# lucagiorgetti/Laplace-DQN-Snake-game

Hardware: NVIDIA B200
Metric: snake_env_steps_per_sec (higher is better)
Workload: dtype u64 bitboards -> f32 obs

## Files before the change

### include/snake_b200.h

```cpp
#ifndef SNAKE_B200_H
#define SNAKE_B200_H

#include <stddef.h>
#include <stdint.h>

#ifdef __cplusplus
extern "C" {
#endif

#define SNK_VERSION 200

#if defined(__GNUC__)
#define SNK_API __attribute__((visibility("default")))
#else
#define SNK_API
#endif

#define SNK_OK 0
#define SNK_ERR_INVALID (-1)
#define SNK_ERR_CUDA (-2)
#define SNK_ERR_NODEVICE (-3)
#define SNK_ERR_UNSUPPORTED (-4)
#define SNK_ERR_TIMEOUT (-5)

// ... 10 lines not shown
#define SNK_OBS_BITS 5

typedef struct snk_env *snk_handle;

SNK_API int snk_create(snk_handle *out, int64_t n_envs, int device, uint32_t flags);
SNK_API int snk_destroy(snk_handle h);
SNK_API int snk_reset(snk_handle h);
SNK_API int snk_set_food_list_host(snk_handle h, const uint8_t *cells_rc_host, int n);
SNK_API int snk_default_food_list_host(uint8_t *cells_rc_host , int *n);
SNK_API int snk_set_stream(snk_handle h, void *cuda_stream);
SNK_API int snk_use_own_stream(snk_handle h);
SNK_API int snk_get_stream(snk_handle h, void **cuda_stream);
SNK_API int snk_set_seed(snk_handle h, uint64_t seed);
SNK_API int snk_sync(snk_handle h);
SNK_API int64_t snk_num_envs(snk_handle h);
SNK_API const char *snk_last_error(void);
SNK_API int snk_version(void);

SNK_API int snk_available_actions(snk_handle h, uint8_t *dirs_3xN);
SNK_API int snk_available_actions_host(snk_handle h, uint8_t *dirs_3xN_host);

SNK_API int snk_step(snk_handle h, const uint8_t *act_idx, float *reward, uint8_t *done);
SNK_API int snk_step_abs(snk_handle h, const uint8_t *dir, float *reward, uint8_t *done);

SNK_API int snk_step_fused(snk_handle h, const float *q, float eps, const float *u, const uint8_t *ridx,
                   uint8_t *act_idx, float *reward, uint8_t *done, void *obs, int obs_fmt,
                   uint8_t *mask, float *ep_return, int32_t *ep_score);
SNK_API int snk_step_fused_host(snk_handle h, const float *q, float eps, const float *u, const uint8_t *ridx,
                        uint8_t *act_idx, float *reward, uint8_t *done, void *obs, int obs_fmt,
                        uint8_t *mask, float *ep_return, int32_t *ep_score);
SNK_API int snk_rollout_fused(snk_handle h, const uint8_t *act_TxN, int64_t T, int is_abs, float *reward, uint8_t *done,
                              void *obs, int obs_fmt, uint8_t *mask, float *ep_return, int32_t *ep_score);
SNK_API int snk_debug_rollout_timing(long long *device_buf);
SNK_API int snk_host_alloc(void **p, size_t bytes);
SNK_API int snk_host_free(void *p);
#define SNK_ALLOC_COMPRESSIBLE 1u
SNK_API int snk_device_alloc(void **p, size_t bytes, int device, uint32_t flags, int *compressible);
SNK_API int snk_device_free(void *p);
SNK_API int snk_compression_supported(int device, int *yes);

SNK_API int snk_state(snk_handle h, void *obs, int obs_fmt);
SNK_API int snk_state_host(snk_handle h, void *obs_host, int obs_fmt);
SNK_API int snk_patch_reset_obs(snk_handle h, const uint8_t *done, void *obs, int obs_fmt);

SNK_API int snk_losing_mask(snk_handle h, uint8_t *mask_3xN);
SNK_API int snk_losing_mask_host(snk_handle h, uint8_t *mask_3xN_host);

SNK_API int snk_select_action(snk_handle h, const float *q_3xN, float eps, const float *u, const uint8_t *ridx,
                      uint8_t *act_idx_out);

SNK_API int snk_masked_target(const float *q_next_3xB, const uint8_t *mask_3xB, const float *r, const uint8_t *done,
                      double gamma, float fill, double *y_f64, float *y_f32, int64_t B, void *cuda_stream);

SNK_API int snk_get_score(snk_handle h, int32_t *score);
SNK_API int snk_get_done(snk_handle h, uint8_t *done);
SNK_API int snk_get_error_flags(snk_handle h, uint8_t *flags);
SNK_API int snk_get_steps(snk_handle h, int32_t *steps);
SNK_API int snk_get_score_host(snk_handle h, int32_t *score_host);
SNK_API int snk_get_done_host(snk_handle h, uint8_t *done_host);
SNK_API int snk_get_error_flags_host(snk_handle h, uint8_t *flags_host);
SNK_API int snk_get_steps_host(snk_handle h, int32_t *steps_host);
SNK_API int snk_count_errors_host(snk_handle h, int64_t *count);

SNK_API int snk_env_checkpoint_bytes(snk_handle h, size_t *bytes);
SNK_API int snk_env_save_host(snk_handle h, void *blob_host, size_t bytes);
SNK_API int snk_env_load_host(snk_handle h, const void *blob_host, size_t bytes, int64_t *first_bad_env);
// ... 105 lines not shown
```

### laplace-dqn-snake-game_b200/__init__.py

```python
import ctypes as C
import os
import warnings

import torch

_HERE = os.path.dirname(os.path.abspath(__file__))
LIB_PATH = os.environ.get("SNAKE_B200_LIB", os.path.join(_HERE, "libsnake_b200.so"))

OBS_NONE, OBS_F32, OBS_I8, OBS_I64, OBS_PACKED2, OBS_BITS = 0, 1, 2, 3, 4, 5
AUTO_RESET = 1
ENV_ERR_FOOD, ENV_ERR_ACTION = 1, 2
_OBS = {
    "f32": (OBS_F32, torch.float32, 200), "i8": (OBS_I8, torch.int8, 200),
    "i64": (OBS_I64, torch.int64, 200), "packed2": (OBS_PACKED2, torch.uint8, 50),
    "bits": (OBS_BITS, torch.uint8, 24),
}


def _obs_shape(fmt, lead):
    per = _OBS[fmt][2]
    return (*lead, 2, 10, 10) if per == 200 else (*lead, per)


def _fmt_code(out):
# ... 44 lines not shown
U, D, L, R = 0, 1, 2, 3
DIRS = ((-1, 0), (1, 0), (0, -1), (0, 1))


class SnakeB200Error(RuntimeError):
    pass


_lib = None


def lib():
    global _lib
    if _lib is not None:
        return _lib
    if not os.path.exists(LIB_PATH):
        raise SnakeB200Error(
            "%s not found: run `python -c 'import __graft_entry__ as g; g.build()'` (needs nvcc). "
            "There is no CPU fallback." % LIB_PATH)
    L = C.CDLL(LIB_PATH)
    vp, i64, u32, i32, f32, f64 = C.c_void_p, C.c_int64, C.c_uint32, C.c_int, C.c_float, C.c_double
    sig = {
        "snk_create": [C.POINTER(vp), i64, i32, u32],
        "snk_destroy": [vp], "snk_reset": [vp], "snk_sync": [vp],
        "snk_set_food_list_host": [vp, vp, i32],
        "snk_default_food_list_host": [vp, C.POINTER(i32)],
        "snk_set_stream": [vp, vp], "snk_use_own_stream": [vp], "snk_get_stream": [vp, C.POINTER(vp)],
        "snk_set_seed": [vp, C.c_uint64],
        "snk_available_actions": [vp, vp],
        "snk_step": [vp, vp, vp, vp], "snk_step_abs": [vp, vp, vp, vp],
        "snk_step_fused": [vp, vp, f32, vp, vp, vp, vp, vp, vp, i32, vp, vp, vp],
        "snk_step_fused_host": [vp, vp, f32, vp, vp, vp, vp, vp, vp, i32, vp, vp, vp],
        "snk_rollout_fused": [vp, vp, i64, i32, vp, vp, vp, i32, vp, vp, vp],
        "snk_host_alloc": [C.POINTER(vp), C.c_size_t], "snk_host_free": [vp],
        "snk_device_alloc": [C.POINTER(vp), C.c_size_t, i32, u32, C.POINTER(i32)], "snk_device_free": [vp],
        "snk_compression_supported": [i32, C.POINTER(i32)],
        "snk_state": [vp, vp, i32], "snk_losing_mask": [vp, vp],
        "snk_state_host": [vp, vp, i32], "snk_losing_mask_host": [vp, vp], "snk_available_actions_host": [vp, vp],
        "snk_patch_reset_obs": [vp, vp, vp, i32],
        "snk_get_score_host": [vp, vp], "snk_get_done_host": [vp, vp], "snk_get_error_flags_host": [vp, vp],
        "snk_get_steps_host": [vp, vp],
        "snk_step_fused_store_host": [vp, vp, vp, f32, vp, vp, vp, vp, vp, vp, i32, vp, vp, vp],
        "snk_replay_gather_host": [vp, vp, i64, vp, vp, vp, vp, vp, vp, vp],
        "snk_select_action": [vp, vp, f32, vp, vp, vp],
        "snk_masked_target": [vp, vp, vp, vp, f64, f32, vp, vp, i64, vp],
        "snk_get_score": [vp, vp], "snk_get_done": [vp, vp], "snk_get_error_flags": [vp, vp],
        "snk_get_steps": [vp, vp], "snk_count_errors_host": [vp, C.POINTER(i64)],
        "snk_env_checkpoint_bytes": [vp, C.POINTER(C.c_size_t)], "snk_env_save_host": [vp, vp, C.c_size_t],
        "snk_env_load_host": [vp, vp, C.c_size_t, C.POINTER(i64)],
        "snk_replay_checkpoint_bytes": [vp, C.POINTER(C.c_size_t)], "snk_replay_save_host": [vp, vp, C.c_size_t],
        "snk_replay_load_host": [vp, vp, C.c_size_t, C.POINTER(i64)],
        "snk_center_columns": [vp, i64, i64, vp, vp, vp],
        "snk_d_store_snapshot": [vp, i64, i64, i64, vp, vp],
        "snk_laplace_sample_weights": [vp, vp, vp, i64, i64, vp, vp, vp, vp],
        "snk_replay_create": [C.POINTER(vp), i64, i32], "snk_replay_destroy": [vp], "snk_replay_clear": [vp],
        "snk_replay_length": [vp, C.POINTER(i64), C.POINTER(i64)],
        "snk_step_fused_store": [vp, vp, vp, f32, vp, vp, vp, vp, vp, vp, i32, vp, vp, vp],
        "snk_replay_gather": [vp, vp, i64, vp, vp, vp, vp, vp, vp, vp, vp, vp],
        "snk_replay_sample_indices": [vp, C.c_uint64, i64, vp, vp],
        "snk_replay_bad_index_host": [vp, C.POINTER(i32)],
        "snk_qnet_create": [C.POINTER(vp), vp, i64, i32, i32], "snk_qnet_destroy": [vp],
        "snk_qnet_forward": [vp, vp, i64, vp, vp], "snk_qnet_precision": [vp, C.POINTER(i32)],
        "snk_qnet_overflow_host": [vp, C.POINTER(i32)], "snk_qnet_debug_timing": [vp, vp],
        "snk_qnet_sample_grads": [vp, vp, vp, vp, i64, vp, vp, i64, vp, i64, vp, vp],
        "snk_qnet_train_step": [vp, vp, vp, vp, i64, vp, f64, f64, f64, vp, vp, vp],
        "snk_qnet_set_params": [vp, vp, vp], "snk_qnet_params": [vp, C.POINTER(vp)],
# ... 496 lines not shown
```

### laplace-dqn-snake-game_b200/csrc/snake_env.cu

```cuda
#include <stdarg.h>
#include <string.h>

#include <new>
#include <mutex>
#include <type_traits>
#include <unordered_map>

#include <cuda.h>

#include "common.h"
#include "sm100.h"

#ifndef SNK_OBS_STORE_MODE
#define SNK_OBS_STORE_MODE 1
#endif
#if SNK_OBS_STORE_MODE == 1
#define SNK_OBS_STORE(p, v) (*(p) = (v))
#elif SNK_OBS_STORE_MODE == 2
#define SNK_OBS_STORE(p, v) __stwt((p), (v))
#else
#define SNK_OBS_STORE(p, v) __stcs((p), (v))
#endif

namespace snk {

static thread_local char g_err[512];
char *err_buf() { return g_err; }
int fail(int code, const char *fmt, ...) {
    va_list ap;
    va_start(ap, fmt);
    vsnprintf(g_err, sizeof(g_err), fmt, ap);
    va_end(ap);
    return code;
}

#ifndef SNK_TPB
#define SNK_TPB 256
#endif
#ifndef SNK_MINB
#define SNK_MINB 1
#endif
#ifndef SNK_UNROLL
#define SNK_UNROLL 4
#endif
constexpr int PHASE_B_UNROLL = SNK_UNROLL;
constexpr int TPB = SNK_TPB;
constexpr int MAX_FOOD = 64;
constexpr int PLANE_WORDS = 16;

constexpr int M_HR = 0, M_HC = 4, M_TR = 8, M_TC = 12, M_FR = 16, M_FC = 20, M_PFR = 24, M_PFC = 28;
constexpr int M_PD = 32, M_LEN = 34, M_T = 41, M_DONE = 51, M_ERR = 52;

constexpr u64 wall_bits(int lo_hi) {
    u64 lo = 0, hi = 0;
    for (int c = 0; c < 10; c++)
        for (int r = 0; r < 10; r++)
            if (r == 0 || r == 9 || c == 0 || c == 9) {
                int k = r + 10 * c;
                if (k < 64) lo |= 1ull << k; else hi |= 1ull << (k - 64);
            }
    return lo_hi ? hi : lo;
}
constexpr u64 WALL_LO = wall_bits(0), WALL_HI = wall_bits(1);

constexpr u64 INIT_OCC = (1ull << (6 + 0)) | (1ull << (7 + 0));
constexpr u64 INIT_MISC = (7ull << M_HR) | (1ull << M_HC) | (8ull << M_TR) | (1ull << M_TC) | (3ull << M_FR) |
                          (4ull << M_FC) | (3ull << M_PFR) | (4ull << M_PFC) | (0ull << M_PD) | (2ull << M_LEN);

struct FoodTable {
    uint8_t bit[MAX_FOOD];
    int n;
    __host__ __device__ u64 mask() const { return n >= 64 ? ~0ull : ((1ull << n) - 1ull); }
};
// ... 8 lines not shown
        case SNK_OBS_F32: return 800;
        case SNK_OBS_I8: return 200;
        case SNK_OBS_I64: return 1600;
        case SNK_OBS_PACKED2: return 50;
        case SNK_OBS_BITS: return 24;
        default: return 0;
    }
}

struct StepOutputs {
    float *reward;
    uint8_t *done;
    void *obs;
    uint8_t *mask;
    float *ep_return;
    int32_t *ep_score;
};

struct StepArgs {
    EnvState s;
    const uint8_t *act;
    const float *q;
    const float *u;
    const uint8_t *ridx;
    float eps;
    uint8_t *act_out;
    StepOutputs out;
    long long env_begin, env_end;
    u64 seed, step_counter;
    int auto_reset, is_abs;
    uint4 *sink;
    long long sink_base, sink_cap, sink_n;
    FoodTable food;
};

constexpr int REC_U4 = 8;

__host__ __device__ __forceinline__ u64 splitmix64(u64 x) {
    x += 0x9E3779B97F4A7C15ull;
    x = (x ^ (x >> 30)) * 0xBF58476D1CE4E5B9ull;
    x = (x ^ (x >> 27)) * 0x94D049BB133111EBull;
    return x ^ (x >> 31);
}

__device__ __forceinline__ void dir_delta(int d, int &dr, int &dc) {
    int s = (d & 1) ? 1 : -1;
    dr = (d & 2) ? 0 : s;
    dc = (d & 2) ? s : 0;
}
__device__ __forceinline__ int av_dir(int prev_dir, int idx) { return idx + (idx >= (prev_dir ^ 1) ? 1 : 0); }

__device__ __forceinline__ int chain_get(u64 lo, u64 hi, int i) {
    int pos = 2 * i;
    return (int)(((pos < 64) ? (lo >> pos) : (hi >> (pos - 64))) & 3ull);
}

__device__ __forceinline__ int food_search(u64 blocked, u64 cons, u64 list_mask, const uint8_t *s_food_bit) {
    if (~blocked == 0ull) return -2;
    u64 cand = ~cons & list_mask;
    while (cand) {
        int i = __ffsll((long long)cand) - 1;
        if (!((blocked >> s_food_bit[i]) & 1ull)) return i;
        cand &= cand - 1;
    }
    return -1;
}

// ... 9 lines not shown
    int best = 0;
    float qb = q0;
    if (jl_isless(qb, q1)) { best = 1; qb = q1; }
    if (jl_isless(qb, q2)) { best = 2; }
    return best;
}
__device__ __forceinline__ void internal_draw(u64 seed, u64 step, long long env, float &u, int &ridx) {
    u64 x = splitmix64(seed ^ splitmix64((u64)env * 0x100000001B3ull + step));
    u = (float)(x >> 40) * 5.9604644775390625e-08f;
    ridx = (int)((x & 0xFFFFFFull) % 3ull);
}

__device__ __forceinline__ void to_full(u64 occ, u64 &lo, u64 &hi) {
    u64 b0 = occ & 0xFF, b1 = (occ >> 8) & 0xFF, b2 = (occ >> 16) & 0xFF, b3 = (occ >> 24) & 0xFF;
    u64 b4 = (occ >> 32) & 0xFF, b5 = (occ >> 40) & 0xFF, b6 = (occ >> 48) & 0xFF, b7 = occ >> 56;
    lo = (b0 << 11) | (b1 << 21) | (b2 << 31) | (b3 << 41) | (b4 << 51) | (b5 << 61);
    hi = (b5 >> 3) | (b6 << 7) | (b7 << 17);
}
__device__ __forceinline__ void set_k(int r, int c, u64 &lo, u64 &hi) {
    int k = r + 10 * c;
    u64 b = 1ull << (k & 63);
    if (k < 64) lo |= b; else hi |= b;
}
__device__ __forceinline__ void board_bits(u64 occ, int fr, int fc, bool has_head, int hr, int hc, u64 &p0lo, u64 &p0hi,
                                           u64 &p1lo, u64 &p1hi) {
    u64 slo, shi;
    to_full(occ, slo, shi);
    if (has_head) set_k(hr, hc, slo, shi);
    u64 flo = WALL_LO, fhi = WALL_HI;
    if (fr != 0) set_k(fr, fc, flo, fhi);
    p0lo = slo | WALL_LO; p0hi = shi | WALL_HI;
    p1lo = flo & ~slo; p1hi = fhi & ~shi;
}
__device__ __forceinline__ u64 spread_nibbles(uint32_t x) {
    u64 v = x;
    v = (v | (v << 16)) & 0x0000FFFF0000FFFFull;
    v = (v | (v << 8)) & 0x00FF00FF00FF00FFull;
    v = (v | (v << 4)) & 0x0F0F0F0F0F0F0F0Full;
    return v;
}
__device__ __forceinline__ u64 unit_bytes(uint32_t p0, uint32_t p1) {
    const uint32_t ev = (p0 & 0x0F0F0F0Fu) | ((p1 << 4) & 0xF0F0F0F0u);
    const uint32_t od = ((p0 >> 4) & 0x0F0F0F0Fu) | (p1 & 0xF0F0F0F0u);
    return (u64)__byte_perm(ev, od, 0x5140) | ((u64)__byte_perm(ev, od, 0x7362) << 32);
}
template <bool PERM>
__device__ __forceinline__ u64 unit_word(uint32_t p0, uint32_t p1) {
    return PERM ? unit_bytes(p0, p1) : (spread_nibbles(p0) | (spread_nibbles(p1) << 4));
}
template <bool PERM = true>
__device__ __forceinline__ void board_planes(u64 occ, int fr, int fc, bool has_head, int hr, int hc, uint32_t *dst) {
    u64 p0lo, p0hi, p1lo, p1hi;
    board_bits(occ, fr, fc, has_head, hr, hc, p0lo, p0hi, p1lo, p1hi);
    u64 *d = reinterpret_cast<u64 *>(dst);
    d[0] = unit_word<PERM>((uint32_t)p0lo, (uint32_t)p1lo);
    d[1] = unit_word<PERM>((uint32_t)(p0lo >> 32), (uint32_t)(p1lo >> 32));
    d[2] = unit_word<PERM>((uint32_t)p0hi, (uint32_t)p1hi);
    d[3] = unit_word<PERM>((uint32_t)(p0hi >> 32), (uint32_t)(p1hi >> 32));
}
__device__ __forceinline__ void board_planes_reg(u64 occ, int fr, int fc, bool has_head, int hr, int hc, uint4 &a, uint4 &b) {
    u64 p0lo, p0hi, p1lo, p1hi;
    board_bits(occ, fr, fc, has_head, hr, hc, p0lo, p0hi, p1lo, p1hi);
    a = make_uint4((uint32_t)p0lo, (uint32_t)(p0lo >> 32), (uint32_t)p0hi, (uint32_t)(p0hi >> 32));
    b = make_uint4((uint32_t)p1lo, (uint32_t)(p1lo >> 32), (uint32_t)p1hi, (uint32_t)(p1hi >> 32));
}

__device__ __forceinline__ int cell_code(const uint32_t *pl, int k) {
    const uint32_t b = reinterpret_cast<const uint8_t *>(pl)[k >> 2];
    const int j = k & 3;
    return (int)(((b >> j) & 1u) | (((b >> (4 + j)) & 1u) << 1));
}
__device__ __forceinline__ int code_value(int code) { return code == 3 ? -1 : code; }

struct ObsTables {
    float4 f32[256];
};
template <int OBS>
__device__ __forceinline__ void fill_tables(ObsTables &tb, int tid, int nt = TPB) {
    if (OBS == SNK_OBS_F32 || OBS == SNK_OBS_I8 || OBS == SNK_OBS_PACKED2) {
        for (int i = tid; i < 256; i += nt) {
            int n0 = i & 15, n1 = i >> 4;
            float v[4];
            uint32_t bytes = 0, packed = 0;
            for (int j = 0; j < 4; j++) {
                int code = ((n0 >> j) & 1) | (((n1 >> j) & 1) << 1);
                v[j] = (float)code_value(code);
                bytes |= (uint32_t)(uint8_t)(int8_t)code_value(code) << (8 * j);
                packed |= (uint32_t)code << (2 * j);
            }
            if (OBS == SNK_OBS_F32) tb.f32[i] = make_float4(v[0], v[1], v[2], v[3]);
            else if (OBS == SNK_OBS_I8) reinterpret_cast<uint32_t *>(tb.f32)[i] = bytes;
// ... 107 lines not shown
            }
        }
        m |= (lose ? 1u : 0u) << k;
    }
    return m;
}

__device__ __forceinline__ void store_mask3(uint8_t *m, uint32_t m3) {
    m[0] = (uint8_t)(m3 & 1u); m[1] = (uint8_t)((m3 >> 1) & 1u); m[2] = (uint8_t)((m3 >> 2) & 1u);
}
__device__ __forceinline__ void store_step_outputs(const StepOutputs &o, long long i, float reward, int done, uint32_t m3, float ret,
                                                   int score) {
    if (o.reward != nullptr) o.reward[i] = reward;
    if (o.done != nullptr) o.done[i] = (uint8_t)done;
    if (o.mask != nullptr) store_mask3(o.mask + 3 * i, m3);
    if (o.ep_return != nullptr) o.ep_return[i] = ret;
    if (o.ep_score != nullptr) o.ep_score[i] = score;
}

constexpr int CHI_FROM_LEN = 32;
struct Env {
    u64 occ, pocc, clo, chi, cons;
    float ret;
    int hr, hc, tr, tc, fr, fc, pfr, pfc, pd, len, t, dn, err;
};
__device__ __forceinline__ void env_unpack(Env &e, u64 misc) {
    e.hr = (int)(misc >> M_HR) & 15; e.hc = (int)(misc >> M_HC) & 15;
    e.tr = (int)(misc >> M_TR) & 15; e.tc = (int)(misc >> M_TC) & 15;
    e.fr = (int)(misc >> M_FR) & 15; e.fc = (int)(misc >> M_FC) & 15;
    e.pfr = (int)(misc >> M_PFR) & 15; e.pfc = (int)(misc >> M_PFC) & 15;
    e.pd = (int)(misc >> M_PD) & 3; e.len = (int)(misc >> M_LEN) & 127; e.t = (int)(misc >> M_T) & 1023;
    e.dn = (int)(misc >> M_DONE) & 1; e.err = (int)(misc >> M_ERR) & 15;
}
template <bool POCC_ALWAYS = true, bool CHI_LAZY = false>
__device__ __forceinline__ void env_load(Env &e, const EnvState &s, long long i) {
    e.occ = s.occ[i]; e.clo = s.clo[i]; e.cons = s.cons[i]; e.ret = s.ret[i];
    const u64 misc = s.misc[i];
    e.pocc = (POCC_ALWAYS || ((misc >> M_DONE) & 1ull)) ? s.pocc[i] : 0ull;
    e.chi = (!CHI_LAZY || ((int)(misc >> M_LEN) & 127) >= CHI_FROM_LEN) ? s.chi[i] : 0ull;
    env_unpack(e, misc);
}
__device__ __forceinline__ void env_store(const Env &e, const EnvState &s, long long i, bool store_chi = true, bool store_cons = true) {
    const u64 misc = ((u64)e.hr << M_HR) | ((u64)e.hc << M_HC) | ((u64)e.tr << M_TR) | ((u64)e.tc << M_TC) |
                     ((u64)e.fr << M_FR) | ((u64)e.fc << M_FC) | ((u64)e.pfr << M_PFR) | ((u64)e.pfc << M_PFC) |
                     ((u64)e.pd << M_PD) | ((u64)e.len << M_LEN) | ((u64)e.t << M_T) | ((u64)e.dn << M_DONE) |
                     ((u64)e.err << M_ERR);
    s.occ[i] = e.occ; s.pocc[i] = e.pocc; s.clo[i] = e.clo; s.misc[i] = misc;
    if (store_chi) s.chi[i] = e.chi;
    if (store_cons) s.cons[i] = e.cons;
    s.ret[i] = e.ret;
}
__device__ __forceinline__ void env_reset(Env &e) {
    e.occ = INIT_OCC; e.pocc = INIT_OCC; e.clo = 0; e.chi = 0; e.cons = 0; e.ret = 0.0f;
    e.hr = 7; e.hc = 1; e.tr = 8; e.tc = 1; e.fr = 3; e.fc = 4; e.pfr = 3; e.pfc = 4; e.pd = 0; e.len = 2; e.t = 0; e.dn = 0;
}
template <bool WITH_MASK = true>
__device__ __forceinline__ float env_advance(Env &e, int &aidx, int is_abs, u64 list_mask, const uint8_t *s_food_bit,
                                             uint32_t &m3) {
    int d;
    if (is_abs) {
        d = aidx;
        if (d > 3) { e.err |= SNK_ENV_ERR_ACTION; d = 0; }
    } else {
        if (aidx > 2) { e.err |= SNK_ENV_ERR_ACTION; aidx = 0; }
        d = av_dir(e.pd, aidx);
    }
    int dr, dc;
    dir_delta(d, dr, dc);
    const int nr = e.hr + dr, nc = e.hc + dc;
    const bool wall = (nr == 0) | (nr == 9) | (nc == 0) | (nc == 9);
    const u64 nbit = wall ? 0ull : (1ull << ((nr - 1) + 8 * (nc - 1)));
    const bool eat = (e.fr != 0) & (nr == e.fr) & (nc == e.fc);
// ... 17 lines not shown
        }
        e.occ |= nbit;
    } else {
        e.occ &= ~(1ull << ((e.tr - 1) + 8 * (e.tc - 1)));
        int c = chain_get(e.clo, e.chi, e.len - 2), er, ec;
        dir_delta(c, er, ec);
        e.tr += er; e.tc += ec;
        e.len--;
        reward = -0.01f;
        self = (e.occ & nbit) != 0ull;
        e.occ |= nbit;
    }
    e.t++;
    const bool lost = wall | self | reverse | (e.t >= 500);
    if (lost) reward = -1.0f;
    e.hr = nr; e.hc = nc; e.pd = d; e.dn = lost;
    e.ret += reward;
    m3 = 7u;
    if (WITH_MASK && !lost) m3 = losing_mask3(e.occ, e.cons, e.hr, e.hc, e.tr, e.tc, e.fr, e.fc, e.pd, e.t, list_mask, s_food_bit, e.err);
    return reward;
}

__device__ __forceinline__ void store_bits_record(void *obs, long long env, u64 pocc, int pfr, int pfc, u64 occ, int fr, int fc,
                                                  int hr, int hc, uint32_t m3, bool done, int aidx, float reward) {
    u64 *rec = reinterpret_cast<u64 *>(obs) + 3 * env;
    const uint32_t cells = (uint32_t)(pfr | (pfc << 4)) | ((uint32_t)(fr | (fc << 4)) << 8) | ((uint32_t)(hr | (hc << 4)) << 16) |
                           (((m3 & 7u) | ((uint32_t)done << 3) | (((uint32_t)aidx & 3u) << 4)) << 24);
    rec[0] = pocc;
    rec[1] = occ;
    rec[2] = (u64)cells | ((u64)__float_as_uint(reward) << 32);
}
__host__ __device__ constexpr bool obs_expands(int fmt) { return fmt != SNK_OBS_NONE && fmt != SNK_OBS_BITS; }

template <int OBS, bool SELECT, bool SINK>
__global__ void __launch_bounds__(TPB, (OBS == SNK_OBS_F32 || OBS == SNK_OBS_I64) ? SNK_MINB : 4) k_step(const __grid_constant__ StepArgs a) {
    __shared__ __align__(16) uint32_t s_planes[TPB * PLANE_WORDS];
    __shared__ ObsTables s_tb;
    __shared__ uint8_t s_food_bit[MAX_FOOD];

    const int tid = threadIdx.x;
    const long long env0 = a.env_begin + (long long)blockIdx.x * TPB;
    const long long rem = a.env_end - env0;
    const int n_local = rem < TPB ? (int)rem : TPB;
    const long long env = env0 + tid;

    if (tid < MAX_FOOD) s_food_bit[tid] = a.food.bit[tid];
    if (obs_expands(OBS)) fill_tables<OBS>(s_tb, tid);
    __syncthreads();

    if (tid < n_local) {
        Env e;
        env_load<SINK, true>(e, a.s, env);
        const bool chi_live = e.len >= CHI_FROM_LEN;
        const u64 cons_loaded = e.cons;
        const u64 list_mask = a.food.mask();
        const u64 occ_tm2 = e.pocc;
        const int fr_tm2 = e.pfr, fc_tm2 = e.pfc, pd_before = e.pd;

        int aidx;
        if (SELECT) {
            float q0 = a.q[3 * env], q1 = a.q[3 * env + 1], q2 = a.q[3 * env + 2];
            float u;
            int ri;
            if (a.u != nullptr && a.ridx != nullptr) {
                u = a.u[env];
                ri = a.ridx[env];
            } else {
                internal_draw(a.seed, a.step_counter, env, u, ri);
                if (a.u != nullptr) u = a.u[env];
                if (a.ridx != nullptr) ri = a.ridx[env];
            }
            aidx = select_idx(q0, q1, q2, a.eps, u, ri);
            if (a.act_out != nullptr) a.act_out[env] = (uint8_t)aidx;
        } else {
            aidx = a.act[env];
        }

        float reward = 0.0f;
        uint32_t m3 = 7u;
        if (!e.dn) reward = env_advance(e, aidx, a.is_abs, list_mask, s_food_bit, m3);

        if (a.out.reward != nullptr) a.out.reward[env] = reward;
        if (a.out.done != nullptr) a.out.done[env] = (uint8_t)e.dn;
        if (a.out.mask != nullptr) store_mask3(a.out.mask + 3 * env, m3);
        if (a.out.ep_return != nullptr) a.out.ep_return[env] = e.ret;
        if (a.out.ep_score != nullptr) a.out.ep_score[env] = e.len - 2;

        if (obs_expands(OBS)) {
            constexpr bool PERM = OBS != SNK_OBS_F32 && OBS != SNK_OBS_I64;
            board_planes<PERM>(e.pocc, e.pfr, e.pfc, false, 0, 0, s_planes + tid * PLANE_WORDS);
            board_planes<PERM>(e.occ, e.fr, e.fc, true, e.hr, e.hc, s_planes + tid * PLANE_WORDS + 8);
        }
        if (OBS == SNK_OBS_BITS)
            store_bits_record(a.out.obs, env, e.pocc, e.pfr, e.pfc, e.occ, e.fr, e.fc, e.hr, e.hc, m3, e.dn, aidx, reward);

        if (SINK) {
            const long long k = env - a.env_begin;
            if (k + a.sink_cap >= a.sink_n) {
                uint4 *rec = a.sink + ((a.sink_base + k) % a.sink_cap) * REC_U4;
                uint4 p0, p1;
                board_planes_reg(occ_tm2, fr_tm2, fc_tm2, false, 0, 0, p0, p1);
                rec[0] = p0; rec[1] = p1;
                board_planes_reg(e.pocc, e.pfr, e.pfc, false, 0, 0, p0, p1);
                rec[2] = p0; rec[3] = p1;
                board_planes_reg(e.occ, e.fr, e.fc, true, e.hr, e.hc, p0, p1);
                rec[4] = p0; rec[5] = p1;
                rec[6] = make_uint4(__float_as_uint(reward),
                                    (uint32_t)aidx | ((uint32_t)e.dn << 8) | (m3 << 16) | ((uint32_t)pd_before << 24),
                                    __float_as_uint(e.ret), (uint32_t)(e.len - 2));
                rec[7] = make_uint4((uint32_t)env, (uint32_t)e.t, 0u, 0u);
            }
        }

        if (e.dn && a.auto_reset) env_reset(e);
        env_store(e, a.s, env, chi_live || e.len >= CHI_FROM_LEN, e.cons != cons_loaded);
    }

    if (obs_expands(OBS)) {
        __syncthreads();
        expand_obs<OBS>(a.out.obs, env0, n_local, s_planes, s_tb, tid);
    }
}

struct RolloutArgs {
    EnvState s;
    const uint8_t *act;
    StepOutputs out;
    long long n;
    int steps, auto_reset, is_abs;
    long long *prof;
    FoodTable food;
};
#ifndef SNK_RTPB
#define SNK_RTPB 128
#endif
#ifndef SNK_WS_EPB
#define SNK_WS_EPB 16
#endif
constexpr int WS_EPB = SNK_WS_EPB;
constexpr int RTPB = SNK_RTPB;
template <int OBS, int EPB>
__global__ void __launch_bounds__(RTPB) k_rollout(const __grid_constant__ RolloutArgs a) {
    __shared__ __align__(16) uint32_t s_planes[EPB * PLANE_WORDS];
    __shared__ ObsTables s_tb;
    __shared__ uint8_t s_food_bit[MAX_FOOD];
    const int tid = threadIdx.x;
    const long long env0 = (long long)blockIdx.x * EPB;
    const long long rem = a.n - env0;
    const int n_local = rem < EPB ? (int)rem : EPB;
    const long long env = env0 + tid;
    const bool mine = tid < n_local;
    if (tid < MAX_FOOD) s_food_bit[tid] = a.food.bit[tid];
    if (OBS != SNK_OBS_NONE) fill_tables<OBS>(s_tb, tid, RTPB);
    __syncthreads();
// ... 532 lines not shown
static cudaError_t ensure(T **p, size_t bytes) {
    if (*p != nullptr) return cudaSuccess;
    return cudaMalloc((void **)p, bytes);
}

static int staging_guard(snk_handle h) {
    SNK_CUDA(cudaStreamWaitEvent(h->stream, h->ev_done, 0));
    return SNK_OK;
}

static int ensure_obs_staging(snk_handle h, size_t bytes) {
    if (h->d_obs_bytes >= bytes) return SNK_OK;
    if (h->d_obs) { SNK_CUDA(cudaStreamSynchronize(h->stream)); SNK_CUDA(cudaFree(h->d_obs)); h->d_obs = nullptr; h->d_obs_bytes = 0; }
    SNK_CUDA(cudaMalloc(&h->d_obs, bytes));
    h->d_obs_bytes = bytes;
    return SNK_OK;
}

template <class Run>
static int get_host(snk_handle h, void *out_host, size_t bytes, Run &&run) {
    int rc = staging_guard(h);
    if (rc == SNK_OK) rc = ensure_obs_staging(h, bytes);
    if (rc == SNK_OK) rc = run(h->d_obs);
    if (rc != SNK_OK) return rc;
    SNK_CUDA(cudaMemcpyAsync(out_host, h->d_obs, bytes, cudaMemcpyDeviceToHost, h->stream));
    SNK_CUDA(cudaStreamSynchronize(h->stream));
    return SNK_OK;
}

#ifndef SNK_HOST_CHUNK_MB
#define SNK_HOST_CHUNK_MB 16u
#endif
static long long *g_rollout_prof = nullptr;

struct Vmm {
    CUresult (*device_get)(CUdevice *, int);
    CUresult (*get_attribute)(int *, CUdevice_attribute, CUdevice);
    CUresult (*granularity)(size_t *, const CUmemAllocationProp *, CUmemAllocationGranularity_flags);
    CUresult (*create)(CUmemGenericAllocationHandle *, size_t, const CUmemAllocationProp *, unsigned long long);
    CUresult (*properties)(CUmemAllocationProp *, CUmemGenericAllocationHandle);
    CUresult (*address_reserve)(CUdeviceptr *, size_t, size_t, CUdeviceptr, unsigned long long);
    CUresult (*map)(CUdeviceptr, size_t, size_t, CUmemGenericAllocationHandle, unsigned long long);
    CUresult (*set_access)(CUdeviceptr, size_t, const CUmemAccessDesc *, size_t);
    CUresult (*unmap)(CUdeviceptr, size_t);
    CUresult (*address_free)(CUdeviceptr, size_t);
    CUresult (*release)(CUmemGenericAllocationHandle);
};
static int vmm_api(const Vmm **out) {
    static Vmm api;
    static int state = 0;
    static std::mutex mu;
    std::lock_guard<std::mutex> lk(mu);
    if (state == 0) {
        struct { const char *name; void **slot; } want[] = {
            {"cuDeviceGet", (void **)&api.device_get}, {"cuDeviceGetAttribute", (void **)&api.get_attribute},
            {"cuMemGetAllocationGranularity", (void **)&api.granularity}, {"cuMemCreate", (void **)&api.create},
            {"cuMemGetAllocationPropertiesFromHandle", (void **)&api.properties},
            {"cuMemAddressReserve", (void **)&api.address_reserve}, {"cuMemMap", (void **)&api.map},
            {"cuMemSetAccess", (void **)&api.set_access}, {"cuMemUnmap", (void **)&api.unmap},
            {"cuMemAddressFree", (void **)&api.address_free}, {"cuMemRelease", (void **)&api.release}};
        state = 1;
        for (auto &w : want) {
            cudaDriverEntryPointQueryResult q;
            if (cudaGetDriverEntryPoint(w.name, w.slot, cudaEnableDefault, &q) != cudaSuccess || q != cudaDriverEntryPointSuccess ||
                *w.slot == nullptr) {
                cudaGetLastError();
// ... 92 lines not shown
    "tail not an interior cell", "food neither an interior cell nor the no-food code", "previous food neither an interior cell nor the no-food code",
    "length outside 2..64", "step count above 500 (499 for a live env)", "consumed food entries outside the food list",
    "previous direction is not the chain's last move", "direction chain leaves the board or crosses itself",
    "direction chain does not end on the tail", "occupancy disagrees with the direction chain"};
static const char *const kReplayRuleText[] = {"", "action index above 2", "done above 1", "mask bits above 7", "previous direction above 3"};

static void env_arrays(const EnvState &s, void *p[7], size_t b[7]) {
    void *q[7] = {s.occ, s.pocc, s.clo, s.chi, s.cons, s.misc, s.ret};
    for (int k = 0; k < 7; k++) { p[k] = q[k]; b[k] = k < 6 ? 8 : 4; }
}

struct LoadScratch {
    uint8_t *p = nullptr;
    ~LoadScratch() { if (p) cudaFree(p); }
    unsigned long long *first() const { return reinterpret_cast<unsigned long long *>(p); }
    uint8_t *data() const { return p + 256; }
};
static int load_scratch(LoadScratch &sc, const void *src_host, size_t bytes, cudaStream_t st) {
    SNK_CUDA(cudaMalloc((void **)&sc.p, 256 + bytes));
    SNK_CUDA(cudaMemsetAsync(sc.p, 0xFF, 8, st));
    if (bytes) SNK_CUDA(cudaMemcpyAsync(sc.data(), src_host, bytes, cudaMemcpyHostToDevice, st));
    return SNK_OK;
}
static int load_verdict(const LoadScratch &sc, cudaStream_t st, long long *idx, int *rule) {
    SNK_CUDA(cudaGetLastError());
    unsigned long long f = 0;
    SNK_CUDA(cudaMemcpyAsync(&f, sc.first(), 8, cudaMemcpyDeviceToHost, st));
    SNK_CUDA(cudaStreamSynchronize(st));
    *idx = f == ~0ull ? -1 : (long long)(f >> 8);
    *rule = (int)(f & 0xFF);
    return SNK_OK;
}

extern "C" {

int snk_debug_rollout_timing(long long *device_buf) {
    g_rollout_prof = device_buf;
    return SNK_OK;
}

int snk_version(void) { return SNK_VERSION; }
const char *snk_last_error(void) { return err_buf(); }

int snk_default_food_list_host(uint8_t *cells_rc_host, int *n) {
    SNK_REQUIRE(cells_rc_host != nullptr && n != nullptr, "null argument");
    memcpy(cells_rc_host, kDefaultFoodRC, 100);
    *n = 50;
    return SNK_OK;
}

int snk_create(snk_handle *out, int64_t n_envs, int device, uint32_t flags) {
    SNK_REQUIRE(out != nullptr, "null out");
    SNK_REQUIRE(n_envs > 0 && n_envs <= (1ll << 31), "n_envs must be in 1..2^31");
    *out = nullptr;
    int ndev = 0;
    cudaError_t e = cudaGetDeviceCount(&ndev);
    if (e != cudaSuccess || ndev == 0)
        return fail(SNK_ERR_NODEVICE, "no CUDA device (%s); libsnake_b200 has no CPU fallback", cudaGetErrorString(e));
    SNK_REQUIRE(device >= 0 && device < ndev, "device index out of range");
    cudaDeviceProp prop;
    SNK_CUDA(cudaGetDeviceProperties(&prop, device));
    if (prop.major != 10)
        return fail(SNK_ERR_NODEVICE, "device %d is sm_%d%d; this library is built for sm_100a only", device, prop.major,
                    prop.minor);
    DeviceGuard guard(device);
    snk_env *h = new (std::nothrow) snk_env();
    if (h == nullptr) return fail(SNK_ERR_INVALID, "out of host memory");
    memset(h, 0, sizeof(*h));
    h->n = n_envs; h->device = device; h->flags = flags; h->seed = 42;
    set_food(h->food, kDefaultFoodRC, 50);
    size_t n = (size_t)n_envs;
// ... 67 lines not shown
    SNK_CUDA(cudaStreamSynchronize(h->stream));
    h->stream = h->own_stream;
    return SNK_OK;
}
int snk_get_stream(snk_handle h, void **cuda_stream) {
    SNK_CHECK_HANDLE(h);
    SNK_REQUIRE(cuda_stream != nullptr, "null out");
    *cuda_stream = (void *)h->stream;
    return SNK_OK;
}
int snk_set_seed(snk_handle h, uint64_t seed) {
    SNK_CHECK_HANDLE(h);
    h->seed = seed; h->step_counter = 0;
    return SNK_OK;
}
int snk_sync(snk_handle h) {
    SNK_CHECK_HANDLE(h);
    SNK_CUDA(cudaStreamSynchronize(h->stream));
    SNK_CUDA(cudaStreamSynchronize(h->copy_stream[0]));
    return SNK_OK;
}
int64_t snk_num_envs(snk_handle h) { return h ? h->n : 0; }

int snk_available_actions(snk_handle h, uint8_t *dirs_3xN) {
    SNK_CHECK_HANDLE(h);
    SNK_REQUIRE(dirs_3xN != nullptr, "null out");
    k_available_actions<<<nblocks(h->n, 256), 256, 0, h->stream>>>(h->s, h->n, dirs_3xN);
    SNK_CUDA(cudaGetLastError());
    return SNK_OK;
}

static int launch_step(StepArgs &a, int obs_fmt, bool select, long long begin, long long end, cudaStream_t st) {
    a.env_begin = begin; a.env_end = end;
    unsigned grid = nblocks(end - begin, TPB);
    if (grid == 0) return SNK_OK;
    return launch_obs_fmt<SNK_OBS_NONE, SNK_OBS_F32, SNK_OBS_I8, SNK_OBS_I64, SNK_OBS_PACKED2, SNK_OBS_BITS>(obs_fmt, [&](auto fmt) {
        constexpr int FMT = decltype(fmt)::value;
        if (a.sink != nullptr) {
            if (select) k_step<FMT, true, true><<<grid, TPB, 0, st>>>(a);
            else k_step<FMT, false, true><<<grid, TPB, 0, st>>>(a);
        } else {
            if (select) k_step<FMT, true, false><<<grid, TPB, 0, st>>>(a);
            else k_step<FMT, false, false><<<grid, TPB, 0, st>>>(a);
        }
    });
}

static StepArgs step_args(snk_handle h, const float *q, float eps, const float *u, const uint8_t *ridx, uint8_t *act_idx,
                          const StepOutputs &out, const snk_replay_s *r) {
    StepArgs a;
    memset(&a, 0, sizeof(a));
    a.s = h->s; a.food = h->food; a.seed = h->seed; a.step_counter = h->step_counter;
    a.auto_reset = (h->flags & SNK_AUTO_RESET) ? 1 : 0;
    a.q = q; a.eps = eps; a.u = u; a.ridx = ridx;
    if (q != nullptr) a.act_out = act_idx; else a.act = act_idx;
    a.out = out;
    if (r != nullptr) { a.sink = r->ring; a.sink_base = r->total; a.sink_cap = r->capacity; a.sink_n = h->n; }
    return a;
}

static int step_plain(snk_handle h, const uint8_t *act, int is_abs, float *reward, uint8_t *done) {
    StepArgs a = step_args(h, nullptr, 0.0f, nullptr, nullptr, nullptr, {reward, done}, nullptr);
    a.act = act; a.is_abs = is_abs;
    int rc = launch_step(a, SNK_OBS_NONE, false, 0, h->n, h->stream);
    h->step_counter++;
    return rc;
}

int snk_step(snk_handle h, const uint8_t *act_idx, float *reward, uint8_t *done) {
    SNK_CHECK_HANDLE(h);
    SNK_REQUIRE(act_idx != nullptr, "null actions");
    return step_plain(h, act_idx, 0, reward, done);
}

int snk_step_abs(snk_handle h, const uint8_t *dir, float *reward, uint8_t *done) {
    SNK_CHECK_HANDLE(h);
    SNK_REQUIRE(dir != nullptr, "null directions");
    return step_plain(h, dir, 1, reward, done);
// ... 579 lines not shown
```

Measured before the change: 8.880 billion.

## Use persistent CTAs with double-buffered planes to overlap env step and obs expansion

For f32/i64 observation formats, the step kernel now launches up to one resident wave of 128-thread CTAs, each walking a contiguous range of tiles. While a tile's planes are expanded to the wide obs output, the next tile's env state is loaded and stepped into a second shared-memory buffer. The aim is to hide state-load and game-logic latency behind the store-heavy expansion and to raise occupancy (TPB 256->128, min blocks 6). It also drops the nibble-spread plane path in favour of byte_perm everywhere and adds an optional globaltimer timeline probe compiled out by default. The costs are a doubled shared buffer, extra syncs per tile, and a cached occupancy query on the host.

```diff
diff --git a/include/snake_b200.h b/include/snake_b200.h
--- a/include/snake_b200.h
+++ b/include/snake_b200.h
@@ -66,6 +66,7 @@
 SNK_API int snk_rollout_fused(snk_handle h, const uint8_t *act_TxN, int64_t T, int is_abs, float *reward, uint8_t *done,
                               void *obs, int obs_fmt, uint8_t *mask, float *ep_return, int32_t *ep_score);
 SNK_API int snk_debug_rollout_timing(long long *device_buf);
+SNK_API int snk_debug_step_timeline(unsigned long long *device_buf, int64_t ctas);
 SNK_API int snk_host_alloc(void **p, size_t bytes);
 SNK_API int snk_host_free(void *p);
 #define SNK_ALLOC_COMPRESSIBLE 1u
diff --git a/laplace-dqn-snake-game_b200/__init__.py b/laplace-dqn-snake-game_b200/__init__.py
--- a/laplace-dqn-snake-game_b200/__init__.py
+++ b/laplace-dqn-snake-game_b200/__init__.py
@@ -100,6 +100,7 @@
         "snk_step_fused": [vp, vp, f32, vp, vp, vp, vp, vp, vp, i32, vp, vp, vp],
         "snk_step_fused_host": [vp, vp, f32, vp, vp, vp, vp, vp, vp, i32, vp, vp, vp],
         "snk_rollout_fused": [vp, vp, i64, i32, vp, vp, vp, i32, vp, vp, vp],
+        "snk_debug_step_timeline": [vp, i64],
         "snk_host_alloc": [C.POINTER(vp), C.c_size_t], "snk_host_free": [vp],
         "snk_device_alloc": [C.POINTER(vp), C.c_size_t, i32, u32, C.POINTER(i32)], "snk_device_free": [vp],
         "snk_compression_supported": [i32, C.POINTER(i32)],
diff --git a/laplace-dqn-snake-game_b200/csrc/snake_env.cu b/laplace-dqn-snake-game_b200/csrc/snake_env.cu
--- a/laplace-dqn-snake-game_b200/csrc/snake_env.cu
+++ b/laplace-dqn-snake-game_b200/csrc/snake_env.cu
@@ -1,6 +1,8 @@
 #include <stdarg.h>
 #include <string.h>
 
+#include <algorithm>
+#include <atomic>
 #include <new>
 #include <mutex>
 #include <type_traits>
@@ -35,10 +37,10 @@
 }
 
 #ifndef SNK_TPB
-#define SNK_TPB 256
+#define SNK_TPB 128
 #endif
 #ifndef SNK_MINB
-#define SNK_MINB 1
+#define SNK_MINB 6
 #endif
 #ifndef SNK_UNROLL
 #define SNK_UNROLL 4
@@ -113,7 +115,28 @@
     uint4 *sink;
     long long sink_base, sink_cap, sink_n;
     FoodTable food;
+#ifdef SNK_STEP_TIMELINE
+    unsigned long long *timeline;
+#endif
 };
+
+constexpr int TL_SLOTS = 64;
+__device__ __forceinline__ void tl_stamp(const StepArgs &a, int slot, unsigned long long value = ~0ull) {
+#ifdef SNK_STEP_TIMELINE
+    if (a.timeline != nullptr && threadIdx.x == 0 && slot < TL_SLOTS) {
+        unsigned long long t = value;
+        if (value == ~0ull) asm volatile("mov.u64 %0, %%globaltimer;" : "=l"(t));
+        a.timeline[(size_t)blockIdx.x * TL_SLOTS + slot] = t;
+    }
+#endif
+}
+__device__ __forceinline__ void tl_end(const StepArgs &a, int tiles) {
+#ifdef SNK_STEP_TIMELINE
+    __syncthreads();
+    tl_stamp(a, 1);
+    tl_stamp(a, 2, (unsigned long long)tiles);
+#endif
+}
 
 constexpr int REC_U4 = 8;
 
@@ -189,31 +212,19 @@
     p0lo = slo | WALL_LO; p0hi = shi | WALL_HI;
     p1lo = flo & ~slo; p1hi = fhi & ~shi;
 }
-__device__ __forceinline__ u64 spread_nibbles(uint32_t x) {
-    u64 v = x;
-    v = (v | (v << 16)) & 0x0000FFFF0000FFFFull;
-    v = (v | (v << 8)) & 0x00FF00FF00FF00FFull;
-    v = (v | (v << 4)) & 0x0F0F0F0F0F0F0F0Full;
-    return v;
-}
 __device__ __forceinline__ u64 unit_bytes(uint32_t p0, uint32_t p1) {
     const uint32_t ev = (p0 & 0x0F0F0F0Fu) | ((p1 << 4) & 0xF0F0F0F0u);
     const uint32_t od = ((p0 >> 4) & 0x0F0F0F0Fu) | (p1 & 0xF0F0F0F0u);
     return (u64)__byte_perm(ev, od, 0x5140) | ((u64)__byte_perm(ev, od, 0x7362) << 32);
 }
-template <bool PERM>
-__device__ __forceinline__ u64 unit_word(uint32_t p0, uint32_t p1) {
-    return PERM ? unit_bytes(p0, p1) : (spread_nibbles(p0) | (spread_nibbles(p1) << 4));
-}
-template <bool PERM = true>
 __device__ __forceinline__ void board_planes(u64 occ, int fr, int fc, bool has_head, int hr, int hc, uint32_t *dst) {
     u64 p0lo, p0hi, p1lo, p1hi;
     board_bits(occ, fr, fc, has_head, hr, hc, p0lo, p0hi, p1lo, p1hi);
     u64 *d = reinterpret_cast<u64 *>(dst);
-    d[0] = unit_word<PERM>((uint32_t)p0lo, (uint32_t)p1lo);
-    d[1] = unit_word<PERM>((uint32_t)(p0lo >> 32), (uint32_t)(p1lo >> 32));
-    d[2] = unit_word<PERM>((uint32_t)p0hi, (uint32_t)p1hi);
-    d[3] = unit_word<PERM>((uint32_t)(p0hi >> 32), (uint32_t)(p1hi >> 32));
+    d[0] = unit_bytes((uint32_t)p0lo, (uint32_t)p1lo);
+    d[1] = unit_bytes((uint32_t)(p0lo >> 32), (uint32_t)(p1lo >> 32));
+    d[2] = unit_bytes((uint32_t)p0hi, (uint32_t)p1hi);
+    d[3] = unit_bytes((uint32_t)(p0hi >> 32), (uint32_t)(p1hi >> 32));
 }
 __device__ __forceinline__ void board_planes_reg(u64 occ, int fr, int fc, bool has_head, int hr, int hc, uint4 &a, uint4 &b) {
     u64 p0lo, p0hi, p1lo, p1hi;
@@ -387,12 +398,11 @@
     e.pd = (int)(misc >> M_PD) & 3; e.len = (int)(misc >> M_LEN) & 127; e.t = (int)(misc >> M_T) & 1023;
     e.dn = (int)(misc >> M_DONE) & 1; e.err = (int)(misc >> M_ERR) & 15;
 }
-template <bool POCC_ALWAYS = true, bool CHI_LAZY = false>
 __device__ __forceinline__ void env_load(Env &e, const EnvState &s, long long i) {
     e.occ = s.occ[i]; e.clo = s.clo[i]; e.cons = s.cons[i]; e.ret = s.ret[i];
     const u64 misc = s.misc[i];
-    e.pocc = (POCC_ALWAYS || ((misc >> M_DONE) & 1ull)) ? s.pocc[i] : 0ull;
-    e.chi = (!CHI_LAZY || ((int)(misc >> M_LEN) & 127) >= CHI_FROM_LEN) ? s.chi[i] : 0ull;
+    e.pocc = s.pocc[i];
+    e.chi = s.chi[i];
     env_unpack(e, misc);
 }
 __device__ __forceinline__ void env_store(const Env &e, const EnvState &s, long long i, bool store_chi = true, bool store_cons = true) {
@@ -476,94 +486,140 @@
 }
 __host__ __device__ constexpr bool obs_expands(int fmt) { return fmt != SNK_OBS_NONE && fmt != SNK_OBS_BITS; }
 
+struct StepIn {
+    u64 occ, clo, cons, misc, pocc;
+    float ret, q0, q1, q2, u;
+    int act;
+};
+template <bool SELECT, bool SINK>
+__device__ __forceinline__ void step_load(StepIn &in, const StepArgs &a, long long env) {
+    in.occ = a.s.occ[env]; in.clo = a.s.clo[env]; in.cons = a.s.cons[env]; in.misc = a.s.misc[env]; in.ret = a.s.ret[env];
+    if (SINK) in.pocc = a.s.pocc[env];
+    if (SELECT) {
+        in.q0 = a.q[3 * env]; in.q1 = a.q[3 * env + 1]; in.q2 = a.q[3 * env + 2];
+        if (a.u != nullptr) in.u = a.u[env];
+        if (a.ridx != nullptr) in.act = a.ridx[env];
+    } else {
+        in.act = a.act[env];
+    }
+}
+
 template <int OBS, bool SELECT, bool SINK>
-__global__ void __launch_bounds__(TPB, (OBS == SNK_OBS_F32 || OBS == SNK_OBS_I64) ? SNK_MINB : 4) k_step(const __grid_constant__ StepArgs a) {
-    __shared__ __align__(16) uint32_t s_planes[TPB * PLANE_WORDS];
+__device__ __forceinline__ void step_env(const StepArgs &a, long long env, const StepIn &in, uint32_t *planes,
+                                         const uint8_t *s_food_bit) {
+    Env e;
+    e.occ = in.occ; e.clo = in.clo; e.cons = in.cons; e.ret = in.ret;
+    e.pocc = SINK ? in.pocc : ((in.misc >> M_DONE) & 1ull) ? a.s.pocc[env] : 0ull;
+    e.chi = ((int)(in.misc >> M_LEN) & 127) >= CHI_FROM_LEN ? a.s.chi[env] : 0ull;
+    env_unpack(e, in.misc);
+    const bool chi_live = e.len >= CHI_FROM_LEN;
+    const u64 cons_loaded = e.cons;
+    const u64 list_mask = a.food.mask();
+    const u64 occ_tm2 = e.pocc;
+    const int fr_tm2 = e.pfr, fc_tm2 = e.pfc, pd_before = e.pd;
+
+    int aidx;
+    if (SELECT) {
+        float u;
+        int ri;
+        if (a.u != nullptr && a.ridx != nullptr) {
+            u = in.u;
+            ri = in.act;
+        } else {
+            internal_draw(a.seed, a.step_counter, env, u, ri);
+            if (a.u != nullptr) u = in.u;
+            if (a.ridx != nullptr) ri = in.act;
+        }
+        aidx = select_idx(in.q0, in.q1, in.q2, a.eps, u, ri);
+        if (a.act_out != nullptr) a.act_out[env] = (uint8_t)aidx;
+    } else {
+        aidx = in.act;
+    }
+
+    float reward = 0.0f;
+    uint32_t m3 = 7u;
+    if (!e.dn) reward = env_advance(e, aidx, a.is_abs, list_mask, s_food_bit, m3);
+
+    if (a.out.reward != nullptr) a.out.reward[env] = reward;
+    if (a.out.done != nullptr) a.out.done[env] = (uint8_t)e.dn;
+    if (a.out.mask != nullptr) store_mask3(a.out.mask + 3 * env, m3);
+    if (a.out.ep_return != nullptr) a.out.ep_return[env] = e.ret;
+    if (a.out.ep_score != nullptr) a.out.ep_score[env] = e.len - 2;
+
+    if (obs_expands(OBS)) {
+        board_planes(e.pocc, e.pfr, e.pfc, false, 0, 0, planes);
+        board_planes(e.occ, e.fr, e.fc, true, e.hr, e.hc, planes + 8);
+    }
+    if (OBS == SNK_OBS_BITS)
+        store_bits_record(a.out.obs, env, e.pocc, e.pfr, e.pfc, e.occ, e.fr, e.fc, e.hr, e.hc, m3, e.dn, aidx, reward);
+
+    if (SINK) {
+        const long long k = env;
+        if (k + a.sink_cap >= a.sink_n) {
+            uint4 *rec = a.sink + ((a.sink_base + k) % a.sink_cap) * REC_U4;
+            uint4 p0, p1;
+            board_planes_reg(occ_tm2, fr_tm2, fc_tm2, false, 0, 0, p0, p1);
+            rec[0] = p0; rec[1] = p1;
+            board_planes_reg(e.pocc, e.pfr, e.pfc, false, 0, 0, p0, p1);
+            rec[2] = p0; rec[3] = p1;
+            board_planes_reg(e.occ, e.fr, e.fc, true, e.hr, e.hc, p0, p1);
+            rec[4] = p0; rec[5] = p1;
+            rec[6] = make_uint4(__float_as_uint(reward),
+                                (uint32_t)aidx | ((uint32_t)e.dn << 8) | (m3 << 16) | ((uint32_t)pd_before << 24),
+                                __float_as_uint(e.ret), (uint32_t)(e.len - 2));
+            rec[7] = make_uint4((uint32_t)env, (uint32_t)e.t, 0u, 0u);
+        }
+    }
+
+    if (e.dn && a.auto_reset) env_reset(e);
+    env_store(e, a.s, env, chi_live || e.len >= CHI_FROM_LEN, e.cons != cons_loaded);
+}
+
+__host__ __device__ constexpr bool step_spread(int fmt) { return fmt == SNK_OBS_F32 || fmt == SNK_OBS_I64; }
+
+template <int OBS, bool SELECT, bool SINK>
+__global__ void __launch_bounds__(TPB, step_spread(OBS) ? SNK_MINB : 4) k_step(const __grid_constant__ StepArgs a) {
+    constexpr bool SPREAD = step_spread(OBS);
+    constexpr int BUF = TPB * PLANE_WORDS;
+    __shared__ __align__(16) uint32_t s_planes[(SPREAD ? 2 : 1) * BUF];
     __shared__ ObsTables s_tb;
     __shared__ uint8_t s_food_bit[MAX_FOOD];
 
     const int tid = threadIdx.x;
-    const long long env0 = a.env_begin + (long long)blockIdx.x * TPB;
-    const long long rem = a.env_end - env0;
-    const int n_local = rem < TPB ? (int)rem : TPB;
-    const long long env = env0 + tid;
-
+    tl_stamp(a, 0);
+    long long lo, hi;
+    if (SPREAD) {
+        const long long quads = (a.env_end - a.env_begin + 3) >> 2;
+        lo = a.env_begin + 4 * (quads * blockIdx.x / gridDim.x);
+        hi = min(a.env_begin + 4 * (quads * (blockIdx.x + 1) / gridDim.x), a.env_end);
+    } else {
+        lo = a.env_begin + (long long)blockIdx.x * TPB;
+        hi = min(lo + TPB, a.env_end);
+    }
+    int n_local = (int)min((long long)TPB, hi - lo);
+    StepIn in;
+    if (tid < n_local) step_load<SELECT, SINK>(in, a, lo + tid);
     if (tid < MAX_FOOD) s_food_bit[tid] = a.food.bit[tid];
     if (obs_expands(OBS)) fill_tables<OBS>(s_tb, tid);
     __syncthreads();
-
-    if (tid < n_local) {
-        Env e;
-        env_load<SINK, true>(e, a.s, env);
-        const bool chi_live = e.len >= CHI_FROM_LEN;
-        const u64 cons_loaded = e.cons;
-        const u64 list_mask = a.food.mask();
-        const u64 occ_tm2 = e.pocc;
-        const int fr_tm2 = e.pfr, fc_tm2 = e.pfc, pd_before = e.pd;
-
-        int aidx;
-        if (SELECT) {
-            float q0 = a.q[3 * env], q1 = a.q[3 * env + 1], q2 = a.q[3 * env + 2];
-            float u;
-            int ri;
-            if (a.u != nullptr && a.ridx != nullptr) {
-                u = a.u[env];
-                ri = a.ridx[env];
-            } else {
-                internal_draw(a.seed, a.step_counter, env, u, ri);
-                if (a.u != nullptr) u = a.u[env];
-                if (a.ridx != nullptr) ri = a.ridx[env];
-            }
-            aidx = select_idx(q0, q1, q2, a.eps, u, ri);
-            if (a.act_out != nullptr) a.act_out[env] = (uint8_t)aidx;
-        } else {
-            aidx = a.act[env];
-        }
-
-        float reward = 0.0f;
-        uint32_t m3 = 7u;
-        if (!e.dn) reward = env_advance(e, aidx, a.is_abs, list_mask, s_food_bit, m3);
-
-        if (a.out.reward != nullptr) a.out.reward[env] = reward;
-        if (a.out.done != nullptr) a.out.done[env] = (uint8_t)e.dn;
-        if (a.out.mask != nullptr) store_mask3(a.out.mask + 3 * env, m3);
-        if (a.out.ep_return != nullptr) a.out.ep_return[env] = e.ret;
-        if (a.out.ep_score != nullptr) a.out.ep_score[env] = e.len - 2;
-
-        if (obs_expands(OBS)) {
-            constexpr bool PERM = OBS != SNK_OBS_F32 && OBS != SNK_OBS_I64;
-            board_planes<PERM>(e.pocc, e.pfr, e.pfc, false, 0, 0, s_planes + tid * PLANE_WORDS);
-            board_planes<PERM>(e.occ, e.fr, e.fc, true, e.hr, e.hc, s_planes + tid * PLANE_WORDS + 8);
-        }
-        if (OBS == SNK_OBS_BITS)
-            store_bits_record(a.out.obs, env, e.pocc, e.pfr, e.pfc, e.occ, e.fr, e.fc, e.hr, e.hc, m3, e.dn, aidx, reward);
-
-        if (SINK) {
-            const long long k = env - a.env_begin;
-            if (k + a.sink_cap >= a.sink_n) {
-                uint4 *rec = a.sink + ((a.sink_base + k) % a.sink_cap) * REC_U4;
-                uint4 p0, p1;
-                board_planes_reg(occ_tm2, fr_tm2, fc_tm2, false, 0, 0, p0, p1);
-                rec[0] = p0; rec[1] = p1;
-                board_planes_reg(e.pocc, e.pfr, e.pfc, false, 0, 0, p0, p1);
-                rec[2] = p0; rec[3] = p1;
-                board_planes_reg(e.occ, e.fr, e.fc, true, e.hr, e.hc, p0, p1);
-                rec[4] = p0; rec[5] = p1;
-                rec[6] = make_uint4(__float_as_uint(reward),
-                                    (uint32_t)aidx | ((uint32_t)e.dn << 8) | (m3 << 16) | ((uint32_t)pd_before << 24),
-                                    __float_as_uint(e.ret), (uint32_t)(e.len - 2));
-                rec[7] = make_uint4((uint32_t)env, (uint32_t)e.t, 0u, 0u);
-            }
-        }
-
-        if (e.dn && a.auto_reset) env_reset(e);
-        env_store(e, a.s, env, chi_live || e.len >= CHI_FROM_LEN, e.cons != cons_loaded);
-    }
-
+    if (tid < n_local) step_env<OBS, SELECT, SINK>(a, lo + tid, in, s_planes + tid * PLANE_WORDS, s_food_bit);
+
+    int tiles = 1;
     if (obs_expands(OBS)) {
         __syncthreads();
-        expand_obs<OBS>(a.out.obs, env0, n_local, s_planes, s_tb, tid);
-    }
+        tl_stamp(a, 3);
+        for (long long t0 = lo;; t0 += TPB, tiles++) {
+            const int n_next = SPREAD ? (int)min((long long)TPB, hi - t0 - TPB) : 0;
+            if (tid < n_next) step_load<SELECT, SINK>(in, a, t0 + TPB + tid);
+            expand_obs<OBS>(a.out.obs, t0, n_local, s_planes + ((tiles - 1) & 1) * BUF, s_tb, tid);
+            if (n_next <= 0) break;
+            if (tid < n_next) step_env<OBS, SELECT, SINK>(a, t0 + TPB + tid, in, s_planes + (tiles & 1) * BUF + tid * PLANE_WORDS, s_food_bit);
+            __syncthreads();
+            tl_stamp(a, 3 + tiles);
+            n_local = n_next;
+        }
+    }
+    tl_end(a, tiles);
 }
 
 struct RolloutArgs {
@@ -1162,6 +1218,8 @@
 #define SNK_HOST_CHUNK_MB 16u
 #endif
 static long long *g_rollout_prof = nullptr;
+static unsigned long long *g_step_timeline = nullptr;
+static long long g_step_timeline_ctas = 0;
 
 struct Vmm {
     CUresult (*device_get)(CUdevice *, int);
@@ -1320,11 +1378,50 @@
     return SNK_OK;
 }
 
+template <int FMT, bool SELECT, bool SINK>
+static int launch_k_step(StepArgs &a, unsigned tiles, cudaStream_t st) {
+    unsigned grid = tiles;
+    if (step_spread(FMT)) {
+        static std::atomic<int> resident_cache[64];
+        int dev = 0, resident = 0;
+        SNK_CUDA(cudaGetDevice(&dev));
+        if (dev < 64) resident = resident_cache[dev].load(std::memory_order_relaxed);
+        if (resident == 0) {
+            int per_sm = 0, sms = 0;
+            SNK_CUDA(cudaOccupancyMaxActiveBlocksPerMultiprocessor(&per_sm, k_step<FMT, SELECT, SINK>, TPB, 0));
+            SNK_CUDA(cudaDeviceGetAttribute(&sms, cudaDevAttrMultiProcessorCount, dev));
+            resident = per_sm * sms;
+            if (resident <= 0) return fail(SNK_ERR_CUDA, "k_step: no CTA of %d threads fits on device %d", TPB, dev);
+            if (dev < 64) resident_cache[dev].store(resident, std::memory_order_relaxed);
+        }
+        if (tiles < 2u * (unsigned)resident) grid = std::min((unsigned)resident, tiles);
+    }
+#ifdef SNK_STEP_TIMELINE
+    if (g_step_timeline != nullptr && grid > g_step_timeline_ctas)
+        return fail(SNK_ERR_INVALID, "step timeline buffer holds %lld CTAs, the launch has %u", g_step_timeline_ctas, grid);
+    a.timeline = g_step_timeline;
+#endif
+    k_step<FMT, SELECT, SINK><<<grid, TPB, 0, st>>>(a);
+    return SNK_OK;
+}
+
 extern "C" {
 
 int snk_debug_rollout_timing(long long *device_buf) {
     g_rollout_prof = device_buf;
     return SNK_OK;
+}
+
+int snk_debug_step_timeline(unsigned long long *device_buf, int64_t ctas) {
+#ifdef SNK_STEP_TIMELINE
+    SNK_REQUIRE(device_buf == nullptr || ctas > 0, "need the number of CTAs the buffer holds");
+    g_step_timeline = device_buf;
+    g_step_timeline_ctas = device_buf ? ctas : 0;
+    return SNK_OK;
+#else
+    (void)device_buf; (void)ctas;
+    return fail(SNK_ERR_UNSUPPORTED, "snk_debug_step_timeline: library built without -DSNK_STEP_TIMELINE");
+#endif
 }
 
 int snk_version(void) { return SNK_VERSION; }
@@ -1458,18 +1555,15 @@
 
 static int launch_step(StepArgs &a, int obs_fmt, bool select, long long begin, long long end, cudaStream_t st) {
     a.env_begin = begin; a.env_end = end;
-    unsigned grid = nblocks(end - begin, TPB);
-    if (grid == 0) return SNK_OK;
-    return launch_obs_fmt<SNK_OBS_NONE, SNK_OBS_F32, SNK_OBS_I8, SNK_OBS_I64, SNK_OBS_PACKED2, SNK_OBS_BITS>(obs_fmt, [&](auto fmt) {
+    const unsigned tiles = nblocks(end - begin, TPB);
+    if (tiles == 0) return SNK_OK;
+    int rc = SNK_OK;
+    const int lrc = launch_obs_fmt<SNK_OBS_NONE, SNK_OBS_F32, SNK_OBS_I8, SNK_OBS_I64, SNK_OBS_PACKED2, SNK_OBS_BITS>(obs_fmt, [&](auto fmt) {
         constexpr int FMT = decltype(fmt)::value;
-        if (a.sink != nullptr) {
-            if (select) k_step<FMT, true, true><<<grid, TPB, 0, st>>>(a);
-            else k_step<FMT, false, true><<<grid, TPB, 0, st>>>(a);
-        } else {
-            if (select) k_step<FMT, true, false><<<grid, TPB, 0, st>>>(a);
-            else k_step<FMT, false, false><<<grid, TPB, 0, st>>>(a);
-        }
+        if (a.sink != nullptr) rc = select ? launch_k_step<FMT, true, true>(a, tiles, st) : launch_k_step<FMT, false, true>(a, tiles, st);
+        else rc = select ? launch_k_step<FMT, true, false>(a, tiles, st) : launch_k_step<FMT, false, false>(a, tiles, st);
     });
+    return rc != SNK_OK ? rc : lrc;
 }
 
 static StepArgs step_args(snk_handle h, const float *q, float eps, const float *u, const uint8_t *ridx, uint8_t *act_idx,
```

New measurement: 9.039 billion, median of 6. +1.8%, better.
